# HAHHHD/mllp

Hardware: AMD Instinct MI355X
Metric: LP instances/sec (fwd+bwd) on Netlib batch; achieved HBM GB/s on CSR SpMM (higher is better)
Workload: dtype f32; 1 GPU; netlib_full: BASELINE.json configs[2], 97 instances / 1,074,147 nnz per global batch, one block-diagonal batch per GPU, one Adam step per global batch: fwd + BCE + bwd + gradient all-reduce + Adam, fp32; global_batch=97, instances_rank0=97, nnz_rank0=1074147, hip_graph=False, parallelism=dp1

## Files before the change

include/mllp_hip.h:

```cpp
#ifndef MLLP_HIP_H
#define MLLP_HIP_H

#include <stdint.h>

#ifdef __cplusplus
extern "C" {
#endif

#define MLLP_ABI_VERSION 6
#define MLLP_FEAT 16
#define MLLP_NUM_PARAMS 4721

#define MLLP_OK 0
#define MLLP_EINVAL (-1)
#define MLLP_EHIP (-2)
#define MLLP_ENOMEM (-3)
#define MLLP_ERANGE (-4)

typedef struct mllp_graph mllp_graph_t;

const char* mllp_last_error(void);
int mllp_abi_version(void);


int mllp_graph_create_host(int64_t n_inst, const int64_t* inst_m, const int64_t* inst_n,
                           const int64_t* indptr, const int32_t* indices, const double* values,
                           int32_t tier_wave, int32_t tier_block, mllp_graph_t** out);

int mllp_csr_transpose_device(int64_t n_rows, int64_t n_cols, int64_t nnz, const int32_t* d_ptr, const int32_t* d_idx,
                              const float* d_val, int32_t* d_t_ptr, int32_t* d_t_idx, float* d_t_val, void* stream);

int mllp_graph_create_device(int64_t n_inst, const int64_t* inst_ptr_m, const int64_t* inst_ptr_n,
                             int64_t nnz,
                             const int32_t* d_csr_ptr, const int32_t* d_csr_idx, const float* d_csr_val,
                             const int32_t* d_csc_ptr, const int32_t* d_csc_idx, const float* d_csc_val,
                             int32_t tier_wave, int32_t tier_block, void* stream, mllp_graph_t** out);

int mllp_graph_destroy(mllp_graph_t* g);

int mllp_graph_dims(const mllp_graph_t* g, int64_t dims[12]);

int mllp_graph_export(const mllp_graph_t* g, int which, void* host_dst, int64_t capacity_bytes);

int mllp_graph_set_path(mllp_graph_t* g, int path);

int mllp_set_fused_grid_limit(int64_t workgroups, int64_t* previous);

int mllp_graph_fused_grid(const mllp_graph_t* g, int64_t info[4]);

int mllp_graph_invalidate_inputs(mllp_graph_t* g);

int mllp_graph_set_values(mllp_graph_t* g, const float* d_val, void* stream);
int mllp_graph_set_values_bytes(const mllp_graph_t* g, int64_t* bytes);
int mllp_graph_scale_values(mllp_graph_t* g, const float* d_row_scale, const float* d_col_scale, void* stream);

int mllp_graph_normalize(mllp_graph_t* g, float* d_x1, float* d_x2, float rhs_cap, int flags, float* d_row_scale,
                         float* d_obj_scale, void* stream);
int mllp_normalize_row_tier(int64_t row_nnz, int* tier);

int mllp_graph_plant_basis(mllp_graph_t* g, const int* d_pivot, const float* d_xstar, const float* d_ystar,
                           const float* d_slack, float dominance, float floor, float* d_x1, float* d_x2, float* d_labels,
                           void* stream);
int mllp_lp_certificate_scratch_bytes(const mllp_graph_t* g, int64_t* bytes);
int mllp_lp_certificate(const mllp_graph_t* g, const float* d_x1, const float* d_x2, const float* d_x, const float* d_y,
                        const float* d_basis, float* d_cert, void* d_scratch, void* stream);

int mllp_basis_repair_scratch_bytes(const mllp_graph_t* g, int64_t max_m, int64_t* bytes);
int mllp_basis_repair(const mllp_graph_t* g, const float* d_x1 , const float* d_x2 ,
                      const int32_t* d_order , float tol, int64_t max_m,
                      float* d_basis , int32_t* d_col_of_row ,
                      float* d_x , float* d_y , int32_t* d_status ,
                      float* d_quality , void* d_scratch, void* stream);

int mllp_basis_simplex_scratch_bytes(const mllp_graph_t* g, int64_t max_m, int64_t* bytes);
int mllp_basis_simplex(const mllp_graph_t* g, const float* d_x1 , const float* d_x2 ,
                       const float* d_start , float tol, float ftol, float dtol, float ptol, float dshift,
                       int64_t max_pivots, int64_t max_m, float* d_basis ,
                       int32_t* d_col_of_row , int32_t* d_trace ,
                       int32_t* d_status , void* d_scratch, void* stream);

int mllp_basis_simplex_guarded(const mllp_graph_t* g, const float* d_x1 , const float* d_x2 ,
                               const float* d_start , float tol, float ftol, float dtol, float ptol, float dshift,
                               int64_t max_pivots, int64_t max_m, int64_t refactor_every, int64_t stall_pivots,
                               float* d_basis , int32_t* d_col_of_row ,
                               int32_t* d_trace , int32_t* d_status ,
                               int32_t* d_guard , void* d_scratch, void* stream);

int mllp_lp_pdhg_limits(int64_t limits[2]);
int mllp_lp_pdhg_scratch_bytes(const mllp_graph_t* g, int64_t max_lds_words, int64_t* bytes);
int mllp_lp_pdhg(const mllp_graph_t* g, const float* d_x1 , const float* d_x2 ,
                 const float* d_x0 , const float* d_y0 , int64_t max_iters,
                 int64_t check_every, float eps, float step, float beta, int64_t max_lds_words, float* d_x ,
                 float* d_y , int32_t* d_status , float* d_kkt ,
                 void* d_scratch, void* stream);

int mllp_lp_pdhg_scaled_limits(int64_t limits[3]);
int mllp_lp_pdhg_scaled_scratch_bytes(const mllp_graph_t* g, int64_t max_lds_words, int64_t* bytes);
int mllp_lp_pdhg_scaled(const mllp_graph_t* g, const float* d_x1 , const float* d_x2 ,
                        const float* d_x0 , const float* d_y0 , int64_t max_iters,
// ... 152 lines not shown
```

mllp_amd/_lib.py:

```python
import ctypes
import os
import subprocess
from ctypes import POINTER, c_char_p, c_double, c_float, c_int, c_int32, c_int64, c_uint32, c_void_p

_HERE = os.path.dirname(os.path.abspath(__file__))
LIB_PATH = os.path.join(_HERE, "csrc", "libmllp_hip.so")
HEADER_PATH = os.path.abspath(os.path.join(_HERE, "..", "include", "mllp_hip.h"))

ABI_VERSION = 6

FEAT = 16
CONV_NAMES = ("gconv1_w2s", "gconv1_s2w", "gconv2_w2s", "gconv2_s2w", "gconv3_w2s", "gconv3_s2w")
CONV_CIN = (1, 1, 16, 16, 16, 16)


def conv_param_count(cin):
    return 4 * FEAT * cin + 5 * FEAT


_CONV_OFFSETS = [0]
for _cin in CONV_CIN:
    _CONV_OFFSETS.append(_CONV_OFFSETS[-1] + conv_param_count(_cin))
FC_OFFSET = _CONV_OFFSETS[-1]
NUM_PARAMS = FC_OFFSET + FEAT + 1


def conv_param_slice(conv):
    i = CONV_NAMES.index(conv) if isinstance(conv, str) else range(len(CONV_NAMES))[conv]
    return slice(_CONV_OFFSETS[i], _CONV_OFFSETS[i + 1])


class MllpError(RuntimeError):
    pass


_PROTOTYPES = {
    "mllp_last_error": (c_char_p, []),
    "mllp_abi_version": (c_int, []),
    "mllp_graph_create_host": (c_int, [c_int64, POINTER(c_int64), POINTER(c_int64), POINTER(c_int64),
                                       POINTER(c_int32), POINTER(c_double), c_int32, c_int32,
                                       POINTER(c_void_p)]),
    "mllp_graph_create_device": (c_int, [c_int64, POINTER(c_int64), POINTER(c_int64), c_int64,
                                         c_void_p, c_void_p, c_void_p, c_void_p, c_void_p, c_void_p,
                                         c_int32, c_int32, c_void_p, POINTER(c_void_p)]),
    "mllp_graph_destroy": (c_int, [c_void_p]),
    "mllp_graph_dims": (c_int, [c_void_p, POINTER(c_int64)]),
    "mllp_graph_export": (c_int, [c_void_p, c_int, c_void_p, c_int64]),
    "mllp_graph_set_path": (c_int, [c_void_p, c_int]),
    "mllp_set_fused_grid_limit": (c_int, [c_int64, POINTER(c_int64)]),
    "mllp_graph_fused_grid": (c_int, [c_void_p, POINTER(c_int64)]),
    "mllp_graph_invalidate_inputs": (c_int, [c_void_p]),
    "mllp_graph_set_values": (c_int, [c_void_p, c_void_p, c_void_p]),
    "mllp_graph_set_values_bytes": (c_int, [c_void_p, POINTER(c_int64)]),
    "mllp_graph_scale_values": (c_int, [c_void_p, c_void_p, c_void_p, c_void_p]),
    "mllp_graph_normalize": (c_int, [c_void_p, c_void_p, c_void_p, c_float, c_int, c_void_p, c_void_p, c_void_p]),
    "mllp_normalize_row_tier": (c_int, [c_int64, POINTER(c_int)]),
    "mllp_graph_plant_basis": (c_int, [c_void_p, c_void_p, c_void_p, c_void_p, c_void_p, c_float, c_float, c_void_p, c_void_p,
                                       c_void_p, c_void_p]),
    "mllp_lp_certificate_scratch_bytes": (c_int, [c_void_p, POINTER(c_int64)]),
    "mllp_lp_certificate": (c_int, [c_void_p, c_void_p, c_void_p, c_void_p, c_void_p, c_void_p, c_void_p, c_void_p, c_void_p]),
    "mllp_basis_repair_scratch_bytes": (c_int, [c_void_p, c_int64, POINTER(c_int64)]),
    "mllp_basis_repair": (c_int, [c_void_p, c_void_p, c_void_p, c_void_p, c_float, c_int64, c_void_p, c_void_p, c_void_p, c_void_p,
                                  c_void_p, c_void_p, c_void_p, c_void_p]),
    "mllp_basis_simplex_scratch_bytes": (c_int, [c_void_p, c_int64, POINTER(c_int64)]),
    "mllp_basis_simplex": (c_int, [c_void_p, c_void_p, c_void_p, c_void_p, c_float, c_float, c_float, c_float, c_float, c_int64,
                                   c_int64, c_void_p, c_void_p, c_void_p, c_void_p, c_void_p, c_void_p]),
    "mllp_basis_simplex_guarded": (c_int, [c_void_p, c_void_p, c_void_p, c_void_p, c_float, c_float, c_float, c_float, c_float,
                                           c_int64, c_int64, c_int64, c_int64, c_void_p, c_void_p, c_void_p, c_void_p, c_void_p,
                                           c_void_p, c_void_p]),
    "mllp_lp_pdhg_limits": (c_int, [POINTER(c_int64)]),
    "mllp_lp_pdhg_scratch_bytes": (c_int, [c_void_p, c_int64, POINTER(c_int64)]),
    "mllp_lp_pdhg": (c_int, [c_void_p, c_void_p, c_void_p, c_void_p, c_void_p, c_int64, c_int64, c_float, c_float, c_float, c_int64,
                             c_void_p, c_void_p, c_void_p, c_void_p, c_void_p, c_void_p]),
    "mllp_lp_pdhg_scaled_limits": (c_int, [POINTER(c_int64)]),
    "mllp_lp_pdhg_scaled_scratch_bytes": (c_int, [c_void_p, c_int64, POINTER(c_int64)]),
    "mllp_lp_pdhg_scaled": (c_int, [c_void_p, c_void_p, c_void_p, c_void_p, c_void_p, c_int64, c_int64, c_float, c_float, c_float,
                                    c_int64, c_int32, c_int32, c_float, c_int64, c_void_p, c_void_p, c_void_p, c_void_p, c_void_p,
                                    c_void_p, c_void_p, c_void_p]),
    "mllp_lp_pdhg_halpern_limits": (c_int, [POINTER(c_int64)]),
    "mllp_lp_pdhg_halpern_scratch_bytes": (c_int, [c_void_p, c_int64, POINTER(c_int64)]),
    "mllp_lp_pdhg_halpern": (c_int, [c_void_p, c_void_p, c_void_p, c_void_p, c_void_p, c_int64, c_int64, c_float, c_float, c_float,
                                     c_int64, c_int32, c_int32, c_float, c_int32, c_int64, c_void_p, c_void_p, c_void_p, c_void_p,
                                     c_void_p, c_void_p, c_void_p, c_void_p]),
    "mllp_lp_pdhg_wide_limits": (c_int, [POINTER(c_int64)]),
    "mllp_lp_pdhg_wide_scratch_bytes": (c_int, [c_void_p, c_int64, POINTER(c_int64)]),
    "mllp_lp_pdhg_wide": (c_int, [c_void_p, c_void_p, c_void_p, c_void_p, c_void_p, c_int64, c_int64, c_int64, c_float, c_float,
                                  c_float, c_int64, c_int32, c_int32, c_float, c_int32, c_int64, c_void_p, c_void_p, c_void_p,
                                  c_void_p, c_void_p, c_void_p, c_void_p, c_void_p]),
    "mllp_graph_build_spmm_copy": (c_int, [c_void_p, c_int, c_int, c_void_p]),
    "mllp_graph_drop_spmm_copy": (c_int, [c_void_p, c_int]),
    "mllp_graph_spmm_copy_info": (c_int, [c_void_p, c_int, POINTER(c_int64)]),
    "mllp_graph_export_spmm_copy": (c_int, [c_void_p, c_int, c_int, c_void_p, c_int64]),
    "mllp_graph_build_stream_copy": (c_int, [c_void_p, c_int, c_int, c_int, c_void_p]),
    "mllp_graph_drop_stream_copy": (c_int, [c_void_p, c_int, c_int]),
    "mllp_graph_stream_copy_info": (c_int, [c_void_p, c_int, c_int, POINTER(c_int64)]),
    "mllp_graph_export_stream_copy": (c_int, [c_void_p, c_int, c_int, c_int, c_void_p, c_int64]),
    "mllp_csr_transpose_device": (c_int, [c_int64, c_int64, c_int64, c_void_p, c_void_p, c_void_p, c_void_p, c_void_p,
                                          c_void_p, c_void_p]),
    "mllp_graph_build_tiled": (c_int, [c_void_p, c_int, c_int, c_void_p]),
    "mllp_graph_tiled_info": (c_int, [c_void_p, c_int, c_int, POINTER(c_int64)]),
    "mllp_graph_export_tiled": (c_int, [c_void_p, c_int, c_int, c_int, c_void_p, c_int64, c_void_p]),
    "mllp_spmm_csr_f32": (c_int, [c_void_p, c_int, c_void_p, c_void_p, c_void_p]),
# ... 111 lines not shown
```

mllp_amd/csrc/fused_kernels.hip:

```cpp
#include <algorithm>
#include <vector>

#include "device_utils.h"
#include "host_graph.h"
#include "internal.h"
#include "node_bodies.h"

namespace mllp {

typedef float f32x4m __attribute__((ext_vector_type(4)));

#ifdef MLLP_TIMING_BUILD
static int g_fused_abl = [] {
    const char* e = getenv("MLLP_FUSED_ABL");
    return e ? atoi(e) : 0;
}();
#define FUSED_ABL(bit) ((J.abl & (bit)) != 0)
__device__ unsigned long long g_fused_stamps[8192 * 8];
__device__ unsigned long long g_fused_stamps1[8192 * 8];
#define FUSED_STAMP(k)                                                                      \
    {                                                                                       \
        __builtin_amdgcn_sched_barrier(0);                                                  \
        const unsigned long long now_ = __builtin_amdgcn_s_memtime();                       \
        __builtin_amdgcn_sched_barrier(0);                                                  \
// ... 1022 lines not shown
#pragma unroll
    for (int s = 0; s < 4; ++s) {
#pragma unroll
        for (int i = 0; i < REG; ++i)
            acc[i] = __builtin_amdgcn_mfma_f32_16x16x4f32(stat_a(c, i)[s], stat_b(c, i)[s], acc[i], 0, 0, 0);
    }
#pragma unroll
    for (int i = REG; i < STAT_TILES; ++i) {
        f32x4m a = park_get(park, i - REG, lane);
#pragma unroll
        for (int s = 0; s < 4; ++s) a = __builtin_amdgcn_mfma_f32_16x16x4f32(stat_a(c, i)[s], stat_b(c, i)[s], a, 0, 0, 0);
        park_put(park, i - REG, lane, a);
    }
}

__device__ __forceinline__ void bwd16_row(const BwdJob16& J, const BwdW16& W, const PartTiers& P, const RowSlot& r,
                                          BwdRow& rd, int2& en, int itn, RowSlot& rn, int part,
                                          int lane, float* merge_lds, float* tiles, f32x4m (&acc)[STAT_TILES]) {
    const bool have = r.row >= 0;
    const int n_mine = FUSED_ABL(1) ? 0 : slot_count(r);
    Gather4 gt;
    gather4_issue(J.s, J.x_src, r, n_mine, 0, part, en, gt);
    SlotReq qn = item_request<4>(J.s, P, max(itn, 0), lane);
    if (itn < 0) qn.row = -1;
    const int xpos = (rd.x.x > 0.0f ? 1 : 0) | (rd.x.y > 0.0f ? 2 : 0) | (rd.x.z > 0.0f ? 4 : 0) | (rd.x.w > 0.0f ? 8 : 0);
    float4 g = f4add(rd.ga, rd.gb);
    g = make_float4(rd.h.x > 0.0f ? g.x : 0.0f, rd.h.y > 0.0f ? g.y : 0.0f, rd.h.z > 0.0f ? g.z : 0.0f, rd.h.w > 0.0f ? g.w : 0.0f);
    const float m = rd.ax.y, rinv = rd.ax.z;
    float4 qp;
    float t;
    row16_project(W, tiles + TB_X * TILE, tiles + TB_SC * TILE, rd.x, FUSED_ABL(16), part, lane, qp, t);
    const DstProj p = dst16_project(W, tiles, g, rd.Z, rd.ax.w, rd.ax.x, have, FUSED_ABL(16), part, lane);
    BwdState st = dst16_sweep(J.s, J.x_src, r, n_mine, part, en, gt, qp, p, t, m, rinv);
    if (r.writer && J.rec && !FUSED_ABL(8)) rec_store(J.rec, r.row, part, qp, p.gv, t, m, rinv, p.ge, p.cc);
    rn = slot_make(qn);
    bwd16_fetch(J, rn, part, rd);
    en = first_entries<4>(J.s, rn, part);
    if (!dst16_merge<FW>(st, r.mode, merge_lds, tiles, lane, part)) return;
    if (J.dx_dst && !FUSED_ABL(4)) dst16_dx(W, tiles, st, r, J.dx_dst, J.mask_dx != 0, xpos, part, lane);
    if (FUSED_ABL(2)) return;
    StatCols c;
    dst16_stat_cols(tiles, st, r, FUSED_ABL(64), part, lane, c);
    if (FUSED_ABL(32)) {
        asm volatile("" :: "v"(c.g[0]), "v"(c.dq[1]), "v"(c.sc[2]), "v"(c.x[3]), "v"(c.z[0]), "v"(c.e[1]));
        return;
    }
    stats_accumulate(c, acc, nullptr, lane);
}

__global__ __launch_bounds__(FT) void fused_bwd16_kernel(BwdLaunch16 A) {
    __shared__ BwdW16 Ws_[MAXJOBS];
    __shared__ float merge_lds[FW * 20];
    __shared__ float tiles_[FW * TB_N * TILE];
    const int tid = threadIdx.x, lane = tid & 63, wave = tid >> 6, part = lane & 3;
    for (int j = 0; j < A.n_jobs; ++j) stage_weights<false, true>(Ws_[j], A.job[j].D, A.job[j].p, nullptr, nullptr, tid);
    __syncthreads();
    float* tiles = tiles_ + wave * TB_N * TILE;
    const BlockPart B = block_part();
    for (int j = 0; j < A.n_jobs; ++j) {
        const BwdJob16& J = A.job[j];
        const PartTiers P = J.s.part[B.px];
        f32x4m acc[STAT_TILES];
#pragma unroll
        for (int i = 0; i < STAT_TILES; ++i) acc[i] = splat4(0.0f);
        const RowSlot none = empty_slot();
        for (int k = B.bi; k < P.n_block; k += B.gp) {
            const RowSlot r = block_slot<4>(J.s, P.row0 + k, tid);
            BwdRow rd;
            bwd16_fetch(J, r, part, rd);
            int2 en = first_entries<4>(J.s, r, part);
            RowSlot rn;
            bwd16_row(J, Ws_[j], P, r, rd, en, -1, rn, part, lane, merge_lds, tiles, acc);
        }
        WaveList wl = wave_list(J.s, B.px, B.gw);
        for (int c0 = 0; c0 < wl.L; c0 += 64) {
            wave_list_chunk(wl, c0, lane);
            int it = wave_list_get(wl, 0);
            RowSlot r = it >= 0 ? item_slot<4>(J.s, P, it, lane) : none;
            BwdRow rd;
            bwd16_fetch(J, r, part, rd);
            int2 en = first_entries<4>(J.s, r, part);
            for (int k = 0; it >= 0; ++k) {
                const int itn = wave_list_get(wl, k + 1);
                RowSlot rn;
                bwd16_row(J, Ws_[j], P, r, rd, en, itn, rn, part, lane, merge_lds, tiles, acc);
                r = rn;
                it = itn;
            }
        }
        __syncthreads();
#pragma unroll
        for (int i = 0; i < STAT_TILES; ++i) stats_tile_store(acc[i], i, tiles_, J.stats, tid);
    }
}

struct L3Job {
    FwdJob16 f;
    float* __restrict__ rec;
    float* __restrict__ dx_dst;
    float* __restrict__ stats;
};
struct L3W {
    float BPq[256], BWv[256], BWs[256], BWvT[256], BWsT[256], BPqT[256];
    float pq0[16], Pt[16], Pb[16], bv[16], we[16], bs[16], fcw[16];
    float pt0, fcb;
};

constexpr int L3_REG_TILES = 2;
constexpr int L3_PARK = (STAT_TILES - L3_REG_TILES) * 256;

__device__ __forceinline__ void l3_row(const L3Job& JJ, const L3W& W, const PartTiers& P, const RowSlot& r, const float4& xd_in,
                                       int2& en, int lrow, const SlotReq& q1, int it2, FwdNext& nx, int part, int lane,
                                       float* merge_lds, float* tiles, float* park, HeadAcc& ha, f32x4m (&acc)[L3_REG_TILES]) {
    const FwdJob16& J = JJ.f;
    const bool have = r.row >= 0;
    const bool writer = r.writer;
    const int n_mine = slot_count(r);
    const int2 en0 = en;
    Gather4 gt;
    gather4_issue(J.s, J.x_src, r, n_mine, 0, part, en, gt);
    fwd16_prefetch(J, P, q1, it2, nx, part, lane);
    const float y = J.labels[max(r.row, 0)];
    const float wn = J.inv_n[max(r.row, 0)] * J.inv_batch;
    const float4 xd = have ? xd_in : f4zero();
    const int xpos = (xd.x > 0.0f ? 1 : 0) | (xd.y > 0.0f ? 2 : 0) | (xd.z > 0.0f ? 4 : 0) | (xd.w > 0.0f ? 8 : 0);
    float4 qp;
    float t;
    row16_project(W, tiles + TB_X * TILE, tiles + TB_Z * TILE, xd, false, part, lane, qp, t);
    SoftState st = fwd16_sweep(J.s, J.x_src, r, n_mine, part, en, gt, qp, t);
    fwd16_take(nx);
    en = en0;
    gather4_issue(J.s, J.x_src, r, n_mine, 0, part, en, gt);
    fwd16_merge<1>(st, r.mode, merge_lds, lane, part);
    const FwdOut f = fwd16_epilogue(W, tiles + TB_X * TILE, tiles + TB_Z * TILE, tiles + TB_SC * TILE, st, false, part, lane);
    const float m = st.L > 0.0f ? st.m : 0.0f;
    const float4 fw = lds4(W.fcw + 4 * part);
    const float z = quad_sum(dot4(f.hv, fw)) + W.fcb;
    float4 g = f4zero();
    if (have) {
        const float e = expf(-fabsf(z));
        const float sig = z >= 0.0f ? 1.0f / (1.0f + e) : e / (1.0f + e);
        const float dz = wn * (sig - y);
        g = make_float4(f.hv.x > 0.0f ? dz * fw.x : 0.0f, f.hv.y > 0.0f ? dz * fw.y : 0.0f,
                        f.hv.z > 0.0f ? dz * fw.z : 0.0f, f.hv.w > 0.0f ? dz * fw.w : 0.0f);
        if (writer) {
// ... 262 lines not shown
        dq = fmaf(dl_, E_.y, dq);                                                          \
    }
        MLLP_BWD1_SLOT(k0, E.e0)
        MLLP_BWD1_SLOT(k0 + 1, E.e1)
        MLLP_BWD1_SLOT(k0 + 2, E.e2)
        MLLP_BWD1_SLOT(k0 + 3, E.e3)
        if (__any(k0 + 4 < n_mine)) {
            MLLP_BWD1_SLOT(k0 + 4, E.e4)
            MLLP_BWD1_SLOT(k0 + 5, E.e5)
            MLLP_BWD1_SLOT(k0 + 6, E.e6)
            MLLP_BWD1_SLOT(k0 + 7, E.e7)
        }
#undef MLLP_BWD1_SLOT
        if (more) E = N;
    }
    FUSED_STAMP(2)
    if (r.mode >= 1) {
        ds = shared_sum1(ds, r.mode); dt = shared_sum1(dt, r.mode); dq = shared_sum1(dq, r.mode);
    }
    if (r.mode == 3) {
        const int wave = threadIdx.x >> 6;
        if (lane == 0) *reinterpret_cast<float4*>(merge_lds + wave * 4) = make_float4(ds, dt, dq, 0.0f);
        __syncthreads();
        float a = 0.0f, b = 0.0f, c = 0.0f;
        for (int w = 0; w < FW; ++w) {
            const float4 v = lds4(merge_lds + w * 4);
            a += v.x; b += v.y; c += v.z;
        }
        ds = a; dt = b; dq = c;
        __syncthreads();
        if (threadIdx.x >= 64) return;
    }
    if (writer) {
        accS[0] = fmaf(dq, x, accS[0]);
        accS[1] += dq;
        accS[2] = fmaf(ds, x, accS[2]);
        accS[3] = fmaf(dt, x, accS[3]);
        accS[4] += ds;
        accS[5] += dt;
    }
    FUSED_STAMP(3)
    const int kq = lane >> 4, rr = lane & 15;
    const float* gt = tiles + kq * G1S + rr;
    const float* rt = tiles + 64 * G1S + kq * R1S + rr;
#pragma unroll
    for (int s = 0; s < 16; ++s) {
        const float a = gt[4 * s * G1S];
        const float b = rr < 5 ? rt[4 * s * R1S] : 0.0f;
        accT = __builtin_amdgcn_mfma_f32_16x16x4f32(a, b, accT, 0, 0, 0);
    }
    FUSED_STAMP(4)
}

__global__ __launch_bounds__(FT) void fused_bwd1_kernel(BwdLaunch1 A) {
    __shared__ BwdW1 Ws_[MAXJOBS];
    __shared__ float merge_lds[FW * 4];
    __shared__ float tiles_[FW * TILE1];
    const int tid = threadIdx.x, lane = tid & 63, wave = tid >> 6;
    for (int j = 0; j < A.n_jobs; ++j) {
        const BwdJob1& J = A.job[j];
        BwdW1& W = Ws_[j];
        if (tid < 16) { W.wv[tid] = J.p.Wv[tid]; W.bv[tid] = J.p.bv[tid]; W.we[tid] = J.p.we[tid]; }
        if (tid == 0) { W.pq = J.D[OFF_PQ]; W.pq0 = J.D[OFF_PQ0]; W.pt = J.D[OFF_PT]; W.pt0 = J.D[OFF_PT0]; }
    }
    __syncthreads();
    float* tiles = tiles_ + wave * TILE1;
    const BlockPart B = block_part();
#ifdef MLLP_TIMING_BUILD
    unsigned long long stamp_sum[8] = {0, 0, 0, 0, 0, 0, 0, 0};
    unsigned long long stamp_last = __builtin_amdgcn_s_memtime();
    const unsigned long long stamp_begin = stamp_last;
#define STAMP_ARGS1 , stamp_sum, stamp_last
#else
#define STAMP_ARGS1
#endif
    for (int j = 0; j < A.n_jobs; ++j) {
        const BwdJob1& J = A.job[j];
        const PartTiers P = J.s.part[B.px];
        f32x4m accT = splat4(0.0f);
        float accS[6] = {0.0f, 0.0f, 0.0f, 0.0f, 0.0f, 0.0f};
        for (int k = B.bi; k < P.n_block; k += B.gp)
            bwd1_row(J, Ws_[j], block_slot<1>(J.s, P.row0 + k, tid), lane, merge_lds, tiles, accT, accS STAMP_ARGS1);
        WaveList wl = wave_list(J.s, B.px, B.gw);
        for (int c0 = 0; c0 < wl.L; c0 += 64) {
            wave_list_chunk(wl, c0, lane);
            int it = wave_list_get(wl, 0);
            SlotReq q = item_request<1>(J.s, P, max(it, 0), lane);
            for (int k = 0; it >= 0; ++k) {
                const int itn = wave_list_get(wl, k + 1);
                const RowSlot r = slot_make(q);
                q = item_request<1>(J.s, P, max(itn, 0), lane);
                bwd1_row(J, Ws_[j], r, lane, merge_lds, tiles, accT, accS STAMP_ARGS1);
#ifdef MLLP_TIMING_BUILD
                stamp_sum[7] += 1;
#endif
                it = itn;
            }
        }
        __syncthreads();
        float* red = tiles_;
#pragma unroll
        for (int q = 0; q < 4; ++q) red[wave * 262 + ((lane >> 4) * 4 + q) * 16 + (lane & 15)] = accT[q];
#pragma unroll
        for (int i = 0; i < 6; ++i) {
            const float v = wave_sum(accS[i]);
            if (lane == 0) red[wave * 262 + 256 + i] = v;
        }
        __syncthreads();
        float* dst = J.stats + (size_t)blockIdx.x * STAT_FLOATS;
        for (int i = tid; i < STAT_FLOATS; i += FT) dst[i] = 0.0f;
        __syncthreads();
        if (tid < 262) {
            float v = 0.0f;
            for (int w = 0; w < FW; ++w) v += red[w * 262 + tid];
            const int o = tid >> 4, n = tid & 15;
            if (tid >= 256) {
                const int i = tid - 256;
                const int slot = i == 0 ? 768 : i == 1 ? 1024 : i == 2 ? 1280 : i == 3 ? 1280 + 16 : i == 4 ? 1536 : 1536 + 16;
                dst[slot] = v;
            } else if (n == 0) dst[o * 16] = v;
            else if (n == 1) dst[256 + o * 16] = v;
            else if (n < 5) dst[512 + o * 16 + (n - 2)] = v;
        }
        __syncthreads();
#ifdef MLLP_TIMING_BUILD
        stamp_last = __builtin_amdgcn_s_memtime();
#endif
    }
#ifdef MLLP_TIMING_BUILD
    if (lane == 0) {
        stamp_sum[6] = __builtin_amdgcn_s_memtime() - stamp_begin;
        unsigned long long* d = g_fused_stamps1 + (size_t)(blockIdx.x * FW + wave) * 8;
        for (int k = 0; k < 8; ++k) d[k] = stamp_sum[k];
    }
#endif
#undef STAMP_ARGS1
}

__global__ __launch_bounds__(RT) void fused_head_bwd_kernel(int n, const float* __restrict__ h3, const float* __restrict__ fcw,
                                                            const float* __restrict__ dlogits, const int* __restrict__ perm,
                                                            float* __restrict__ dh3, float* __restrict__ head_part) {
    __shared__ float head_lds[(RT / 64) * 18];
    const int tid = threadIdx.x, lane = tid & 63, part = lane & 3;
    HeadAcc ha;
    ha.w = f4zero(); ha.b = 0.0f; ha.l = 0.0f;
    const float4 fw = ld4(fcw + 4 * part);
    for (int row = blockIdx.x * (RT / 4) + (tid >> 2); row < n; row += gridDim.x * (RT / 4)) {
        const float dz = dlogits[perm[row]];
        const float4 hv = ld4(h3 + (size_t)row * 16 + 4 * part);
        *reinterpret_cast<float4*>(dh3 + (size_t)row * 16 + 4 * part) = f4scale(fw, dz);
        fma4(dz, hv, ha.w);
        if (part == 0) ha.b += dz;
    }
    head_partials_store<RT / 64>(ha, head_lds, head_part, tid);
}

struct ReduceArgs {
    const float* stats[MODEL_CONVS];
    float* out[MODEL_CONVS];
    int nblk;
    const float* head_part;
    float* head_out;
    float* loss_out;
};

__device__ __forceinline__ void fused_reduce_body(const ReduceArgs& A, int n_conv) {
    __shared__ float sh[32][32];
    const int tid = threadIdx.x;
    if ((int)blockIdx.x == n_conv * STAT_TILES) {
        if (!A.head_part) return;
        const int col = tid & 31, slice = tid >> 5;
        float v = 0.0f;
        if (col < 18)
            for (int b = slice; b < A.nblk; b += 32) v += A.head_part[(size_t)b * 18 + col];
        sh[slice][col] = v;
        __syncthreads();
        if (tid < 18) {
            float t = 0.0f;
            for (int q = 0; q < 32; ++q) t += sh[q][tid];
            if (tid < 17) A.head_out[tid] = t;
            else if (A.loss_out) A.loss_out[0] = t;
// ... 321 lines not shown

static BwdJob16 bwd_job16(const FusedOrient& o, const FusedModel& m, int c, const float* x_src, const float* x_dst,
                          const float* h, const float* dh_a, const float* dh_b, float* dx_dst, bool need_rec, bool mask_dx) {
    const ConvWs& w = m.w.c[c];
    BwdJob16 J = {};
    J.s = items_dev(o, 0);
    J.x_src = x_src; J.x_dst = x_dst; J.D = w.derived; J.p = conv_params_at(conv_at(m.P, c), MODEL_CONV[c].cin);
    J.h = h; J.dh_a = dh_a; J.dh_b = dh_b; J.Z = w.Z; J.aux = w.aux;
    J.rec = need_rec ? w.rec : nullptr;
    J.dx_dst = dx_dst;
    J.mask_dx = mask_dx ? 1 : 0;
    J.stats = w.stats;
#ifdef MLLP_TIMING_BUILD
    J.abl = g_fused_abl;
#endif
    return J;
}
static SrcJob16 src_job16(const FusedOrient& o_src_major, const ConvWs& w, const float* x_rows, float* dx, const float* add) {
    SrcJob16 J = {};
    J.s = items_dev(o_src_major, 2);
    J.x = x_rows; J.rec = w.rec; J.dx = dx;
    J.addp = add ? add : x_rows; J.addw = add ? 1.0f : 0.0f; J.mask = 1;
    return J;
}
static BwdJob1 bwd_job1(const FusedOrient& o, const FusedModel& m, int c, const float* x_dst, const float* g_masked) {
    const ConvWs& w = m.w.c[c];
    BwdJob1 J = {};
    J.s = items_dev(o, 1);
    J.x_dst = x_dst; J.D = w.derived; J.p = conv_params_at(conv_at(m.P, c), MODEL_CONV[c].cin);
    J.g = g_masked; J.Z = w.Z; J.aux = w.aux; J.stats = w.stats;
    return J;
}

int fused_backward(const mllp_graph* g, const FusedModel& m, bool premasked, float* grads, float* loss, hipStream_t s,
                   const FusedAdam* adam) {
    const int G = fused_grid(g);
    const ModelWs& w = m.w;
    int rc;
    const FusedOrient& A = g->FA;
    const FusedOrient& At = g->FAt;
    if (premasked) {
        L3Job L = {};
        L.f = l3_fwd_job(g, m, 2);
        L.rec = w.c[CONV_3V].rec; L.dx_dst = w.d2v; L.stats = w.c[CONV_3V].stats;
        hipLaunchKernelGGL(fused_l3_kernel, dim3(G), dim3(FT), 0, s, L);
        if ((rc = check_launch("fused_l3"))) return rc;
    } else {
        BwdLaunch16 L = {};
        L.n_jobs = 1;
        L.job[0] = bwd_job16(At, m, CONV_3V, w.h2c, w.h2v, w.h3v, w.d3v, nullptr, w.d2v, true, true);
        hipLaunchKernelGGL(fused_bwd16_kernel, dim3(G), dim3(FT), 0, s, L);
        if ((rc = check_launch("fused_bwd16 C3"))) return rc;
    }
    {
        SrcLaunch16 S = {};
        S.n_jobs = 1;
        S.job[0] = src_job16(A, w.c[CONV_3V], w.h2c, w.d2c, nullptr);
        hipLaunchKernelGGL(fused_src16_kernel, dim3(2 * G), dim3(FT), 0, s, S);
        if ((rc = check_launch("fused_src16 C3"))) return rc;
        BwdLaunch16 L = {};
        L.n_jobs = 1;
        L.job[0] = bwd_job16(At, m, CONV_2V, w.h1c, w.h1v, nullptr, w.d2v, nullptr, w.d1v, true, true);
        hipLaunchKernelGGL(fused_bwd16_kernel, dim3(G), dim3(FT), 0, s, L);
        if ((rc = check_launch("fused_bwd16 C2V"))) return rc;
    }
    {
        BwdLaunch16 L = {};
        L.n_jobs = 1;
        L.job[0] = bwd_job16(A, m, CONV_2C, w.h1v, w.h1c, nullptr, w.d2c, nullptr, w.d1c, true, true);
        hipLaunchKernelGGL(fused_bwd16_kernel, dim3(G), dim3(FT), 0, s, L);
        if ((rc = check_launch("fused_bwd16 C2C"))) return rc;
        SrcLaunch16 S = {};
        S.n_jobs = 2;
        S.job[0] = src_job16(A, w.c[CONV_2V], w.h1c, w.d1c_b, w.d1c);
        S.job[1] = src_job16(At, w.c[CONV_2C], w.h1v, w.d1v_b, w.d1v);
        hipLaunchKernelGGL(fused_src16_kernel, dim3(2 * G), dim3(FT), 0, s, S);
        if ((rc = check_launch("fused_src16 C2V + C2C"))) return rc;
    }
    {
        BwdLaunch1 L = {};
        L.n_jobs = 2;
        L.job[0] = bwd_job1(A, m, CONV_1C, g->x2_p, w.d1c_b);
        L.job[1] = bwd_job1(At, m, CONV_1V, g->x1_p, w.d1v_b);
        hipLaunchKernelGGL(fused_bwd1_kernel, dim3(G), dim3(FT), 0, s, L);
        if ((rc = check_launch("fused_bwd1"))) return rc;
    }
    ReduceArgs R = {};
    for (int c = 0; c < MODEL_CONVS; ++c) { R.stats[c] = w.c[c].stats; R.out[c] = w.c[c].red; }
    R.nblk = G;
    R.head_part = w.head_partials;
    R.head_out = grads + OFF_FC;
    R.loss_out = loss;
    if (adam) {
        TailArgs T = {};
        T.R = R;
        for (int c = 0; c < MODEL_CONVS; ++c) {
            T.p[c] = conv_params_at(conv_at(m.P, c), MODEL_CONV[c].cin);
            T.cin[c] = MODEL_CONV[c].cin;
            T.grads[c] = conv_at(grads, c);
            T.D[c] = w.c[c].derived;
        }
        T.zero = grads + OFF_UNUSED;
        T.n_zero = LEN_UNUSED;
        T.params = adam->params; T.grads_all = grads; T.m = adam->m; T.v = adam->v; T.state = adam->state;
        T.eps = adam->eps;
        T.n_params = adam->n;
        T.sync = g->tail_sync;
        T.err = g->tail_err_dev;
        if (g->tail_err_host && *(volatile unsigned*)g->tail_err_host != 0u)
            return fail(MLLP_EHIP, "the grid barrier of fused_tail_kernel timed out in an earlier step (the device was shared with "
                                   "other work): parameters and optimizer state since then are invalid; recreate the graph");
        hipLaunchKernelGGL(fused_tail_kernel, dim3(MODEL_CONVS * STAT_TILES + 1), dim3(RT), 0, s, T, MODEL_CONVS);
        return check_launch("fused_tail");
    }
    {
        hipLaunchKernelGGL(fused_reduce_kernel, dim3(MODEL_CONVS * STAT_TILES + 1), dim3(RT), 0, s, R, MODEL_CONVS);
        if ((rc = check_launch("fused_reduce"))) return rc;
    }
    return model_finalize(g, m.P, w, true, grads, s);
}

}
```

mllp_amd/csrc/graph.cpp:

```cpp
#include <algorithm>
#include <atomic>
#include <cmath>
#include <cstring>

#include "host_graph.h"
#include "internal.h"

namespace mllp {

static thread_local std::string g_err;
void set_error(const std::string& msg) { g_err = msg; }
int fail(int code, const std::string& msg) {
    g_err = msg;
    return code;
}
int hip_fail(hipError_t e, const char* what) {
    g_err = std::string(what) + ": " + hipGetErrorString(e);
    return e == hipErrorOutOfMemory ? MLLP_ENOMEM : MLLP_EHIP;
}
const char* last_error_cstr() { return g_err.c_str(); }

static std::atomic<int64_t> g_fused_grid_limit{0};

template <class T>
static int upload(mllp_graph* g, const T* host, size_t count, T** dev) {
    *dev = nullptr;
    size_t bytes = std::max<size_t>(count, 1) * sizeof(T);
    void* p = nullptr;
    MLLP_HIP_TRY(hipMalloc(&p, bytes));
    g->allocs.push_back(p);
    if (count) MLLP_HIP_TRY(hipMemcpy(p, host, count * sizeof(T), hipMemcpyHostToDevice));
    *dev = static_cast<T*>(p);
    return MLLP_OK;
}

static void choose_tiers(mllp_graph* g) {
    const TierConfig c = host_choose_tiers(g->nnz, g->tier_wave, g->tier_block);
    g->tier_wave = c.tier_wave; g->tier_block = c.tier_block; g->chunk_nnz = c.chunk_nnz;
}

static int build_tiers(mllp_graph* g, Orient& o, const int* h_ptr) {
    HostTiers t;
    TierConfig c;
    c.tier_wave = g->tier_wave; c.tier_block = g->tier_block; c.chunk_nnz = g->chunk_nnz;
    host_build_tiers(h_ptr, o.n_dst, c, &t);
    o.n_group = t.n_group;
    o.tier_wave = g->tier_wave;
    o.short_rows = t.short_rows;
    o.n_wave = (int)t.rows_wave.size();
    o.n_chunk = (int)(t.chunks.size() / 4);
    o.n_split = (int)(t.split.size() / 4);
    o.n_slots = t.n_slots;
    int rc;
    o.rows_group = nullptr;
    if ((rc = upload(g, t.rows_wave.data(), t.rows_wave.size(), &o.rows_wave))) return rc;
    if ((rc = upload(g, t.chunks.data(), t.chunks.size(), &o.chunks))) return rc;
    if ((rc = upload(g, t.split.data(), t.split.size(), &o.split))) return rc;
    return MLLP_OK;
}

static int finish_common(mllp_graph* g) {
    std::vector<float> inv_n((size_t)g->N);
    std::vector<int> ipn(g->n_inst + 1), ipm(g->n_inst + 1);
    g->max_inst_n = 0;
    for (int64_t k = 0; k < g->n_inst; ++k) {
        int64_t a = g->h_inst_ptr_n[k], b = g->h_inst_ptr_n[k + 1];
        for (int64_t i = a; i < b; ++i) inv_n[i] = 1.0f / (float)(b - a);
        g->max_inst_n = std::max<int>(g->max_inst_n, (int)(b - a));
    }
    for (int64_t k = 0; k <= g->n_inst; ++k) {
        ipn[k] = (int)g->h_inst_ptr_n[k];
        ipm[k] = (int)g->h_inst_ptr_m[k];
    }
    int rc;
    for (Orient* o : {&g->A, &g->At}) {
// ... 121 lines not shown
        if (e != hipSuccess) { rc = hip_fail(e, "copy row pointers to host"); break; }
        if (h_rp[0] != 0 || h_cp[0] != 0 || h_rp[M] != nnz || h_cp[N] != nnz) {
            rc = fail(MLLP_EINVAL, "row pointers inconsistent with nnz");
            break;
        }
        if ((rc = build_tiers(g, g->A, h_rp.data()))) break;
        if ((rc = build_tiers(g, g->At, h_cp.data()))) break;
        if ((rc = finish_common(g))) break;
        g->h_csr_ptr = h_rp; g->h_csc_ptr = h_cp;
        if (g->nnz < ((int64_t)32 << 20) && (rc = fused_graph_build(g, h_rp.data(), h_cp.data()))) break;
    } while (0);
    if (rc) {
        std::string keep = mllp_last_error();
        mllp_graph_destroy(g);
        set_error(keep);
        return rc;
    }
    *out = g;
    return MLLP_OK;
}

extern "C" int mllp_graph_destroy(mllp_graph_t* g) {
    if (!g) return MLLP_OK;
    for (mllp::Orient* o : {&g->A, &g->At}) {
        for (mllp::StreamCopy& sc : o->stream) mllp::stream_copy_free(sc);
        mllp::lane_copy_free(o->lane1);
        for (mllp::Tiled& tl : o->tiled) mllp::tiled_free(tl);
    }
    for (void* p : g->allocs) (void)hipFree(p);
    if (g->tail_err_host) (void)hipHostFree(g->tail_err_host);
    for (auto& e : g->ev)
        if (e) (void)hipEventDestroy(e);
    if (g->aux) (void)hipStreamDestroy(g->aux);
    delete g;
    return MLLP_OK;
}

extern "C" int mllp_graph_dims(const mllp_graph_t* g, int64_t dims[12]) {
    if (!g || !dims) return fail(MLLP_EINVAL, "mllp_graph_dims: null argument");
    dims[0] = g->M; dims[1] = g->N; dims[2] = g->nnz; dims[3] = g->n_inst;
    dims[4] = g->A.n_group; dims[5] = g->A.n_wave; dims[6] = g->A.n_chunk;
    dims[7] = g->At.n_group; dims[8] = g->At.n_wave; dims[9] = g->At.n_chunk;
    dims[10] = g->A.n_split; dims[11] = g->At.n_split;
    return MLLP_OK;
}

extern "C" int mllp_set_fused_grid_limit(int64_t workgroups, int64_t* previous) {
    if (workgroups < 0) return fail(MLLP_EINVAL, "mllp_set_fused_grid_limit: the limit must be 0 (none) or a positive number of workgroups");
    const int64_t old = g_fused_grid_limit.exchange(workgroups, std::memory_order_relaxed);
    if (previous) *previous = old;
    return MLLP_OK;
}

extern "C" int mllp_graph_fused_grid(const mllp_graph_t* g, int64_t info[4]) {
    if (!g || !info) return fail(MLLP_EINVAL, "mllp_graph_fused_grid: null argument");
    info[0] = fused_grid(g); info[1] = FUSED_PARTS; info[2] = g->n_cu_dev; info[3] = g->grid_limit;
    return MLLP_OK;
}

extern "C" int mllp_graph_export(const mllp_graph_t* g, int which, void* host_dst, int64_t capacity_bytes) {
    if (!g || !host_dst) return fail(MLLP_EINVAL, "mllp_graph_export: null argument");
    const void* src = nullptr;
    int64_t bytes = 0;
    switch (which) {
        case 0: src = g->A.ptr; bytes = (g->M + 1) * 4; break;
        case 1: src = g->A.idx; bytes = g->nnz * 4; break;
        case 2: src = g->A.val; bytes = g->nnz * 4; break;
        case 3: src = g->At.ptr; bytes = (g->N + 1) * 4; break;
        case 4: src = g->At.idx; bytes = g->nnz * 4; break;
        case 5: src = g->At.val; bytes = g->nnz * 4; break;
        case 6: src = g->inv_n; bytes = g->N * 4; break;
        default: return fail(MLLP_EINVAL, "mllp_graph_export: unknown array id");
    }
    if (capacity_bytes < bytes) return fail(MLLP_EINVAL, "mllp_graph_export: destination too small");
    MLLP_HIP_TRY(hipDeviceSynchronize());
    if (bytes) MLLP_HIP_TRY(hipMemcpy(host_dst, src, bytes, hipMemcpyDeviceToHost));
    return MLLP_OK;
}
```

mllp_amd/csrc/internal.h:

```cpp
#pragma once
#include <hip/hip_runtime.h>
#include <stdint.h>

#include <algorithm>
#include <string>
#include <vector>

#include "../../include/mllp_hip.h"

namespace mllp {

constexpr int FEAT = 16;
constexpr int BLOCK = 256;
constexpr int REC_W = 40;
constexpr int STAT_TILES = 7;
constexpr int STAT_FLOATS = STAT_TILES * 256;
constexpr int STAT_BLOCKS_MAX = 256;

void set_error(const std::string& msg);
int fail(int code, const std::string& msg);
int hip_fail(hipError_t e, const char* what);

#define MLLP_HIP_TRY(expr)                                              \
    do {                                                                \
// ... 320 lines not shown
                float* partials, hipStream_t s);
int launch_head_finalize(const float* partials, int n_blocks, float* grad_fc , float* loss ,
                         hipStream_t s);
int head_blocks_for(int64_t n);
int launch_adam(float* p, const float* g, float* m, float* v, float* state, float eps, float gscale, int64_t n,
                hipStream_t s);
int launch_fill_zero(float* p, int64_t n, hipStream_t s);

constexpr int64_t SMALL_STEP_MAX_NODES = 8192, SMALL_STEP_MAX_NNZ = 16384;
constexpr int SMALL_STEP_THREADS = 1024, SMALL_STEP_LDS_BYTES = 63296;
int launch_small_step(const mllp_graph* g, float* params, const float* x1, const float* x2, const float* labels,
                      float inv_batch, const ModelWs& w, float* logits, float* loss, float* grads, float* m, float* v,
                      float* state, float eps, hipStream_t s);
int launch_topm_metrics(const mllp_graph* g, const float* logits, const float* labels, void* scratch, float* out,
                        hipStream_t s);
int launch_topm_select(const int* ptr_n, const int* ptr_m, int64_t n_seg, int n_dense, int m_dense, const float* logits,
                       unsigned char* mask, int* index, float* stats, hipStream_t s);

constexpr int BASIS_LDS_MAX_M = 192;
constexpr int BASIS_MAX_M = 8192;
__host__ __device__ constexpr int64_t basis_repair_vec_words(int64_t m) { return 4 * m; }
__host__ __device__ constexpr int64_t basis_repair_words(int64_t m) { return m * m; }

constexpr int SIMPLEX_LDS_MAX_M = 192;
constexpr int SIMPLEX_MAX_M = 4096;
__host__ __device__ constexpr int64_t simplex_vec_words(int64_t m) { return 6 * m; }
__host__ __device__ constexpr int64_t simplex_words(int64_t m, int64_t n) {
    return (m > SIMPLEX_LDS_MAX_M ? m * m : 0) + n;
}

constexpr int64_t PDHG_LDS_WORDS = 36864;
constexpr int PDHG_THREADS = 1024;
constexpr int64_t PDHG_SCALED_LDS_WORDS = PDHG_LDS_WORDS;
constexpr int PDHG_SCALED_THREADS = PDHG_THREADS;
constexpr int PDHG_SCALED_MAX_RUIZ = 64;
__host__ __device__ constexpr int64_t pdhg_words(int64_t m, int64_t n) { return 3 * n + 2 * m; }
__host__ __device__ constexpr int64_t pdhg_scaled_side_words(int64_t m, int64_t n) { return 2 * n + 2 * m; }

constexpr int TOPM_LOSS_T = 1024;
constexpr int TOPM_LOSS_LDS_MAX = 16 * TOPM_LOSS_T;
constexpr int TOPM_LOSS_MAX_ITER = 64;

struct FusedModel {
    const float* P;
    const ModelWs& w;
    const float *x1, *x2, *labels;
    float inv_batch;
    float* logits;
};
int model_param_prep(const float* P, const ModelWs& w, hipStream_t s);
int model_finalize(const mllp_graph* g, const float* P, const ModelWs& w, bool reduced, float* grads, hipStream_t s);
int fused_graph_build(mllp_graph* g, const int* h_csr_ptr, const int* h_csc_ptr);
int fused_grid(const mllp_graph* g);
int fused_refill_values(mllp_graph* g, hipStream_t s);
int fused_bind(mllp_graph* g, const float* x1, const float* x2, const float* labels, hipStream_t s);
int fused_forward(mllp_graph* g, const FusedModel& m, int head_mode, hipStream_t s, bool skip_prep = false);
int fused_head_backward(const mllp_graph* g, const FusedModel& m, const float* dlogits, hipStream_t s);
struct FusedAdam {
    float *params, *m, *v, *state;
    float eps;
    int n;
};
int fused_backward(const mllp_graph* g, const FusedModel& m, bool premasked, float* grads, float* loss, hipStream_t s,
                   const FusedAdam* adam = nullptr);
int fused_input_grads(const mllp_graph* g, const FusedModel& m, float* dx1, float* dx2, float* dval, hipStream_t s);

}
```

mllp_amd/graph.py:

```python
import contextlib
import ctypes
import itertools
import math
import time
from ctypes import c_int32, c_int64, c_double, c_void_p
from typing import List, Optional, Sequence

import numpy as np
import torch

from . import _lib
from .data import LPInstance


_B128_GROUPS = [[0, 1, 2, 3, 12, 13, 14, 15, 20, 21, 22, 23, 24, 25, 26, 27],
                [4, 5, 6, 7, 8, 9, 10, 11, 16, 17, 18, 19, 28, 29, 30, 31]]
LANE_GROUPS = [[l + h for l in grp if (l & 3) == r] for h in (0, 32) for grp in _B128_GROUPS for r in range(4)]


def set_fused_grid_limit(n):
    prev = c_int64()
    _lib.check(_lib.lib().mllp_set_fused_grid_limit(int(n), ctypes.byref(prev)))
    return int(prev.value)


@contextlib.contextmanager
def fused_grid_limit(n):
    prev = set_fused_grid_limit(n)
    try:
        yield
    finally:
        set_fused_grid_limit(prev)


def build_tiled_arrays(ptr, idx, val, n_dst, R, CB, variant=0, entry_order="joint"):
    dev, nnz = idx.device, int(idx.numel())
    if nnz == 0:
        return None
    n_tiles = (n_dst + R - 1) // R
    deg = (ptr[1:] - ptr[:-1]).long()
    rows = torch.repeat_interleave(torch.arange(n_dst, device=dev, dtype=torch.int32), deg)
    tile = torch.div(rows, R, rounding_mode="floor")
    blk = torch.div(idx, CB, rounding_mode="floor")
    tl = tile.long()
    lo = torch.full((n_tiles,), 2 ** 30, dtype=torch.int32, device=dev).scatter_reduce(0, tl, blk, "amin")
    hi = torch.full((n_tiles,), -1, dtype=torch.int32, device=dev).scatter_reduce(0, tl, blk, "amax")
    nbt = torch.where(hi >= 0, hi - lo + 1, torch.zeros_like(hi)).long()
    lo = torch.where(hi >= 0, lo, torch.zeros_like(lo))
    tile_blk = torch.zeros(n_tiles + 1, dtype=torch.int64, device=dev)
    tile_blk[1:] = torch.cumsum(nbt, 0)
    n_tb = int(tile_blk[-1])
    max_nbt = int(nbt.max())
    if n_tb * R >= 2 ** 31 - 1 or max_nbt > 255:
        return None
    key = (tile_blk[tl] + (blk - lo[tl]).long()) * R + (rows - tile * R).long()
    del rows, tile, tl
    counts = torch.bincount(key, minlength=n_tb * R)
    lane_fixed = int(variant) == 4
    if lane_fixed and R % 64:
        return None
    if lane_fixed:
        order = torch.arange(R, device=dev).expand(n_tb, R).contiguous()
    else:
        order = torch.argsort(counts.view(n_tb, R), dim=1, descending=True, stable=True)
    inv = torch.empty_like(order)
    inv.scatter_(1, order, torch.arange(R, device=dev).expand(n_tb, R))
    sorted_counts = torch.gather(counts.view(n_tb, R), 1, order).reshape(-1)
    del counts
    ptr2 = torch.zeros(n_tb * R + 1, dtype=torch.int64, device=dev)
    ptr2[1:] = torch.cumsum(sorted_counts, 0)
    del sorted_counts
    max_run = int((ptr2[R::R] - ptr2[:-1:R]).max())
    ar = torch.arange(nnz, device=dev, dtype=torch.int64)
    is_start = torch.ones(nnz, dtype=torch.bool, device=dev)
    is_start[1:] = key[1:] != key[:-1]
    start_idx = torch.cummax(torch.where(is_start, ar, torch.zeros_like(ar)), 0)[0]
    pos_key = torch.div(key, R, rounding_mode="floor") * R + inv.reshape(-1)[key]
    del key, inv, is_start
    cls = ((idx - blk * CB) & 3).long()
    joint = int(variant) in (0, 1, 4) and R % 16 == 0 and entry_order != "perrow"
    if joint:
        n_run = n_tb * R
        cnt = torch.zeros(n_run * 4, dtype=torch.int32, device=dev)
        cnt.index_add_(0, pos_key * 4 + cls, torch.ones(nnz, dtype=torch.int32, device=dev))
        base = torch.cumsum(cnt, 0, dtype=torch.int64) - cnt
# ... 1132 lines not shown
```

Measured before the change: 312,900 instances/s.

## Merge C2V and C2C backward launches and defer per-job stats reductions

The two 16-channel backward jobs for the second conv layer now run in one multi-job launch instead of two sequential launches. Inside the bwd16 and bwd1 kernels, the statistics reduction and store that followed each job (with its block barriers) is deferred to the end. Earlier job accumulators are parked in LDS or registers so the barriers are paid once. A runtime switch restores separate launches. The change removes a launch and intra-kernel sync points, at the cost of extra LDS and register pressure that could reduce occupancy.

```diff
diff --git a/include/mllp_hip.h b/include/mllp_hip.h
--- a/include/mllp_hip.h
+++ b/include/mllp_hip.h
@@ -45,6 +45,8 @@
 int mllp_graph_set_path(mllp_graph_t* g, int path);
 
 int mllp_set_fused_grid_limit(int64_t workgroups, int64_t* previous);
+
+int mllp_set_fused_bwd_split(int on);
 
 int mllp_graph_fused_grid(const mllp_graph_t* g, int64_t info[4]);
 
diff --git a/mllp_amd/_lib.py b/mllp_amd/_lib.py
--- a/mllp_amd/_lib.py
+++ b/mllp_amd/_lib.py
@@ -48,6 +48,7 @@
     "mllp_graph_export": (c_int, [c_void_p, c_int, c_void_p, c_int64]),
     "mllp_graph_set_path": (c_int, [c_void_p, c_int]),
     "mllp_set_fused_grid_limit": (c_int, [c_int64, POINTER(c_int64)]),
+    "mllp_set_fused_bwd_split": (c_int, [c_int]),
     "mllp_graph_fused_grid": (c_int, [c_void_p, POINTER(c_int64)]),
     "mllp_graph_invalidate_inputs": (c_int, [c_void_p]),
     "mllp_graph_set_values": (c_int, [c_void_p, c_void_p, c_void_p]),
diff --git a/mllp_amd/csrc/fused_kernels.hip b/mllp_amd/csrc/fused_kernels.hip
--- a/mllp_amd/csrc/fused_kernels.hip
+++ b/mllp_amd/csrc/fused_kernels.hip
@@ -1098,15 +1098,18 @@
     __shared__ BwdW16 Ws_[MAXJOBS];
     __shared__ float merge_lds[FW * 20];
     __shared__ float tiles_[FW * TB_N * TILE];
+    __shared__ float park_[FW * (STAT_TILES - 1) * 256];
+    static_assert(MAXJOBS == 2, "one parked set of statistics tiles");
     const int tid = threadIdx.x, lane = tid & 63, wave = tid >> 6, part = lane & 3;
     for (int j = 0; j < A.n_jobs; ++j) stage_weights<false, true>(Ws_[j], A.job[j].D, A.job[j].p, nullptr, nullptr, tid);
     __syncthreads();
     float* tiles = tiles_ + wave * TB_N * TILE;
+    float* park = park_ + wave * (STAT_TILES - 1) * 256;
     const BlockPart B = block_part();
+    f32x4m acc[STAT_TILES], kept = splat4(0.0f);
     for (int j = 0; j < A.n_jobs; ++j) {
         const BwdJob16& J = A.job[j];
         const PartTiers P = J.s.part[B.px];
-        f32x4m acc[STAT_TILES];
 #pragma unroll
         for (int i = 0; i < STAT_TILES; ++i) acc[i] = splat4(0.0f);
         const RowSlot none = empty_slot();
@@ -1134,9 +1137,21 @@
                 it = itn;
             }
         }
-        __syncthreads();
-#pragma unroll
-        for (int i = 0; i < STAT_TILES; ++i) stats_tile_store(acc[i], i, tiles_, J.stats, tid);
+        if (j + 1 < A.n_jobs) {
+#pragma unroll
+            for (int i = 0; i < STAT_TILES - 1; ++i) park_put(park, i, lane, acc[i]);
+            kept = acc[STAT_TILES - 1];
+        }
+    }
+    __syncthreads();
+    float* stats = A.job[A.n_jobs - 1].stats;
+#pragma unroll
+    for (int i = 0; i < STAT_TILES; ++i) stats_tile_store(acc[i], i, tiles_, stats, tid);
+    if (A.n_jobs > 1) {
+        stats = A.job[0].stats;
+#pragma unroll
+        for (int i = 0; i < STAT_TILES - 1; ++i) stats_tile_store(park_get(park, i, lane), i, tiles_, stats, tid);
+        stats_tile_store(kept, STAT_TILES - 1, tiles_, stats, tid);
     }
 }
 
@@ -1505,10 +1520,40 @@
     FUSED_STAMP(4)
 }
 
+__device__ __forceinline__ void bwd1_stats_store(const f32x4m& accT, const float (&accS)[6], float* red,
+                                                 float* __restrict__ stats, int tid) {
+    const int lane = tid & 63, wave = tid >> 6;
+#pragma unroll
+    for (int q = 0; q < 4; ++q) red[wave * 262 + ((lane >> 4) * 4 + q) * 16 + (lane & 15)] = accT[q];
+#pragma unroll
+    for (int i = 0; i < 6; ++i) {
+        const float v = wave_sum(accS[i]);
+        if (lane == 0) red[wave * 262 + 256 + i] = v;
+    }
+    __syncthreads();
+    float* dst = stats + (size_t)blockIdx.x * STAT_FLOATS;
+    for (int i = tid; i < STAT_FLOATS; i += FT) dst[i] = 0.0f;
+    __syncthreads();
+    if (tid < 262) {
+        float v = 0.0f;
+        for (int w = 0; w < FW; ++w) v += red[w * 262 + tid];
+        const int o = tid >> 4, n = tid & 15;
+        if (tid >= 256) {
+            const int i = tid - 256;
+            const int slot = i == 0 ? 768 : i == 1 ? 1024 : i == 2 ? 1280 : i == 3 ? 1280 + 16 : i == 4 ? 1536 : 1536 + 16;
+            dst[slot] = v;
+        } else if (n == 0) dst[o * 16] = v;
+        else if (n == 1) dst[256 + o * 16] = v;
+        else if (n < 5) dst[512 + o * 16 + (n - 2)] = v;
+    }
+    __syncthreads();
+}
+
 __global__ __launch_bounds__(FT) void fused_bwd1_kernel(BwdLaunch1 A) {
     __shared__ BwdW1 Ws_[MAXJOBS];
     __shared__ float merge_lds[FW * 4];
     __shared__ float tiles_[FW * TILE1];
+    static_assert(MAXJOBS == 2, "one set of accumulators put aside");
     const int tid = threadIdx.x, lane = tid & 63, wave = tid >> 6;
     for (int j = 0; j < A.n_jobs; ++j) {
         const BwdJob1& J = A.job[j];
@@ -1527,11 +1572,14 @@
 #else
 #define STAMP_ARGS1
 #endif
+    f32x4m accT, keptT = splat4(0.0f);
+    float accS[6], keptS[6] = {0.0f, 0.0f, 0.0f, 0.0f, 0.0f, 0.0f};
     for (int j = 0; j < A.n_jobs; ++j) {
         const BwdJob1& J = A.job[j];
         const PartTiers P = J.s.part[B.px];
-        f32x4m accT = splat4(0.0f);
-        float accS[6] = {0.0f, 0.0f, 0.0f, 0.0f, 0.0f, 0.0f};
+        accT = splat4(0.0f);
+#pragma unroll
+        for (int i = 0; i < 6; ++i) accS[i] = 0.0f;
         for (int k = B.bi; k < P.n_block; k += B.gp)
             bwd1_row(J, Ws_[j], block_slot<1>(J.s, P.row0 + k, tid), lane, merge_lds, tiles, accT, accS STAMP_ARGS1);
         WaveList wl = wave_list(J.s, B.px, B.gw);
@@ -1550,36 +1598,15 @@
                 it = itn;
             }
         }
-        __syncthreads();
-        float* red = tiles_;
-#pragma unroll
-        for (int q = 0; q < 4; ++q) red[wave * 262 + ((lane >> 4) * 4 + q) * 16 + (lane & 15)] = accT[q];
-#pragma unroll
-        for (int i = 0; i < 6; ++i) {
-            const float v = wave_sum(accS[i]);
-            if (lane == 0) red[wave * 262 + 256 + i] = v;
-        }
-        __syncthreads();
-        float* dst = J.stats + (size_t)blockIdx.x * STAT_FLOATS;
-        for (int i = tid; i < STAT_FLOATS; i += FT) dst[i] = 0.0f;
-        __syncthreads();
-        if (tid < 262) {
-            float v = 0.0f;
-            for (int w = 0; w < FW; ++w) v += red[w * 262 + tid];
-            const int o = tid >> 4, n = tid & 15;
-            if (tid >= 256) {
-                const int i = tid - 256;
-                const int slot = i == 0 ? 768 : i == 1 ? 1024 : i == 2 ? 1280 : i == 3 ? 1280 + 16 : i == 4 ? 1536 : 1536 + 16;
-                dst[slot] = v;
-            } else if (n == 0) dst[o * 16] = v;
-            else if (n == 1) dst[256 + o * 16] = v;
-            else if (n < 5) dst[512 + o * 16 + (n - 2)] = v;
-        }
-        __syncthreads();
-#ifdef MLLP_TIMING_BUILD
-        stamp_last = __builtin_amdgcn_s_memtime();
-#endif
-    }
+        if (j + 1 < A.n_jobs) {
+            keptT = accT;
+#pragma unroll
+            for (int i = 0; i < 6; ++i) keptS[i] = accS[i];
+        }
+    }
+    __syncthreads();
+    bwd1_stats_store(accT, accS, tiles_, A.job[A.n_jobs - 1].stats, tid);
+    if (A.n_jobs > 1) bwd1_stats_store(keptT, keptS, tiles_, A.job[0].stats, tid);
 #ifdef MLLP_TIMING_BUILD
     if (lane == 0) {
         stamp_sum[6] = __builtin_amdgcn_s_memtime() - stamp_begin;
@@ -2007,24 +2034,29 @@
         hipLaunchKernelGGL(fused_bwd16_kernel, dim3(G), dim3(FT), 0, s, L);
         if ((rc = check_launch("fused_bwd16 C3"))) return rc;
     }
+    const bool split = fused_bwd_split();
     {
         SrcLaunch16 S = {};
         S.n_jobs = 1;
         S.job[0] = src_job16(A, w.c[CONV_3V], w.h2c, w.d2c, nullptr);
         hipLaunchKernelGGL(fused_src16_kernel, dim3(2 * G), dim3(FT), 0, s, S);
         if ((rc = check_launch("fused_src16 C3"))) return rc;
-        BwdLaunch16 L = {};
-        L.n_jobs = 1;
-        L.job[0] = bwd_job16(At, m, CONV_2V, w.h1c, w.h1v, nullptr, w.d2v, nullptr, w.d1v, true, true);
-        hipLaunchKernelGGL(fused_bwd16_kernel, dim3(G), dim3(FT), 0, s, L);
-        if ((rc = check_launch("fused_bwd16 C2V"))) return rc;
     }
     {
         BwdLaunch16 L = {};
-        L.n_jobs = 1;
-        L.job[0] = bwd_job16(A, m, CONV_2C, w.h1v, w.h1c, nullptr, w.d2c, nullptr, w.d1c, true, true);
-        hipLaunchKernelGGL(fused_bwd16_kernel, dim3(G), dim3(FT), 0, s, L);
-        if ((rc = check_launch("fused_bwd16 C2C"))) return rc;
+        L.n_jobs = 2;
+        L.job[0] = bwd_job16(At, m, CONV_2V, w.h1c, w.h1v, nullptr, w.d2v, nullptr, w.d1v, true, true);
+        L.job[1] = bwd_job16(A, m, CONV_2C, w.h1v, w.h1c, nullptr, w.d2c, nullptr, w.d1c, true, true);
+        for (int j = 0; split && j < 2; ++j) {
+            BwdLaunch16 L1 = {};
+            L1.n_jobs = 1;
+            L1.job[0] = L.job[j];
+            hipLaunchKernelGGL(fused_bwd16_kernel, dim3(G), dim3(FT), 0, s, L1);
+        }
+        if (!split) hipLaunchKernelGGL(fused_bwd16_kernel, dim3(G), dim3(FT), 0, s, L);
+        if ((rc = check_launch("fused_bwd16 C2V + C2C"))) return rc;
+    }
+    {
         SrcLaunch16 S = {};
         S.n_jobs = 2;
         S.job[0] = src_job16(A, w.c[CONV_2V], w.h1c, w.d1c_b, w.d1c);
@@ -2037,7 +2069,13 @@
         L.n_jobs = 2;
         L.job[0] = bwd_job1(A, m, CONV_1C, g->x2_p, w.d1c_b);
         L.job[1] = bwd_job1(At, m, CONV_1V, g->x1_p, w.d1v_b);
-        hipLaunchKernelGGL(fused_bwd1_kernel, dim3(G), dim3(FT), 0, s, L);
+        for (int j = 0; split && j < 2; ++j) {
+            BwdLaunch1 L1 = {};
+            L1.n_jobs = 1;
+            L1.job[0] = L.job[j];
+            hipLaunchKernelGGL(fused_bwd1_kernel, dim3(G), dim3(FT), 0, s, L1);
+        }
+        if (!split) hipLaunchKernelGGL(fused_bwd1_kernel, dim3(G), dim3(FT), 0, s, L);
         if ((rc = check_launch("fused_bwd1"))) return rc;
     }
     ReduceArgs R = {};
diff --git a/mllp_amd/csrc/graph.cpp b/mllp_amd/csrc/graph.cpp
--- a/mllp_amd/csrc/graph.cpp
+++ b/mllp_amd/csrc/graph.cpp
@@ -21,6 +21,8 @@
 const char* last_error_cstr() { return g_err.c_str(); }
 
 static std::atomic<int64_t> g_fused_grid_limit{0};
+static std::atomic<int> g_fused_bwd_split{0};
+bool fused_bwd_split() { return g_fused_bwd_split.load(std::memory_order_relaxed) != 0; }
 
 template <class T>
 static int upload(mllp_graph* g, const T* host, size_t count, T** dev) {
@@ -248,6 +250,8 @@
     return MLLP_OK;
 }
 
+extern "C" int mllp_set_fused_bwd_split(int on) { return g_fused_bwd_split.exchange(on != 0, std::memory_order_relaxed); }
+
 extern "C" int mllp_graph_fused_grid(const mllp_graph_t* g, int64_t info[4]) {
     if (!g || !info) return fail(MLLP_EINVAL, "mllp_graph_fused_grid: null argument");
     info[0] = fused_grid(g); info[1] = FUSED_PARTS; info[2] = g->n_cu_dev; info[3] = g->grid_limit;
diff --git a/mllp_amd/csrc/internal.h b/mllp_amd/csrc/internal.h
--- a/mllp_amd/csrc/internal.h
+++ b/mllp_amd/csrc/internal.h
@@ -396,6 +396,7 @@
 int model_finalize(const mllp_graph* g, const float* P, const ModelWs& w, bool reduced, float* grads, hipStream_t s);
 int fused_graph_build(mllp_graph* g, const int* h_csr_ptr, const int* h_csc_ptr);
 int fused_grid(const mllp_graph* g);
+bool fused_bwd_split();
 int fused_refill_values(mllp_graph* g, hipStream_t s);
 int fused_bind(mllp_graph* g, const float* x1, const float* x2, const float* labels, hipStream_t s);
 int fused_forward(mllp_graph* g, const FusedModel& m, int head_mode, hipStream_t s, bool skip_prep = false);
diff --git a/mllp_amd/graph.py b/mllp_amd/graph.py
--- a/mllp_amd/graph.py
+++ b/mllp_amd/graph.py
@@ -31,6 +31,10 @@
         yield
     finally:
         set_fused_grid_limit(prev)
+
+
+def set_fused_bwd_split(on):
+    return bool(_lib.lib().mllp_set_fused_bwd_split(1 if on else 0))
 
 
 def build_tiled_arrays(ptr, idx, val, n_dst, R, CB, variant=0, entry_order="joint"):
```

After: 315,600 instances/s (median of 5 runs). About the same (+0.8%).
